# imagemagick/ImageMagick

Measured on NVIDIA H100. Metric: Mpixels/s on 8K RGBA Gaussian-blur σ=4 + Lanczos 2×; % HBM roofline, higher is better.
Workload: dtype f64

## Files before the change

### imagemagick_b200/csrc/conv_mma.cu

```cuda
#include "mb200_internal.h"
#include "conv_common.cuh"

#include <cuda_runtime.h>

#include <cstdint>

namespace mb200 {
namespace {

template <int NKS>
struct MmaTaps { double k[4 * NKS]; };

struct MmaArgs {
  const void *src;
  void *dst;
  int width, height;
  int off;
  int ntaps;
  int strip;
  const float *aux;
  double gain, qthreshold;
  int l2pf;
};

__device__ __forceinline__ void dmma(double (&d)[2], double a, double b) {
  asm volatile("mma.sync.aligned.m8n8k4.row.col.f64.f64.f64.f64 {%0,%1}, {%2}, {%3}, {%0,%1};"
      : "+d"(d[0]), "+d"(d[1]) : "d"(a), "d"(b));
}

template <int IO> struct Raw;
template <> struct Raw<0> { float4 a; };
template <> struct Raw<2> { double2 a, b; };

template <int NKS, int AXIS, int IO, int EPI, int MINB>
__global__ void __launch_bounds__(128, MINB) conv_mma_kernel(const MmaArgs a, const MmaTaps<NKS> taps) {
  static_assert(NKS % 2 == 0, "the prologue stages whole 8-position blocks");
  static_assert(EPI == 0 || (AXIS == 1 && IO == 0), "the fused epilogue belongs to the final column pass");
// ... 236 lines not shown
    output(prev, epi_prev, prev_valid);
    if (b > 0) outp += ostep;

    if (window_bad != 0) {
#pragma unroll
      for (int g = 0; g < 2; ++g) {
        double s0 = 0.0, s1 = 0.0, s2 = 0.0, s3 = 0.0;
        int u = 8 * sb + n8;
        if (u >= RR) u -= RR;
        for (int t = 0; t < a.ntaps; ++t) {
          const double *p = ring + static_cast<unsigned>(u) * kUStride + lane_px_off + g * kGroup;
          const double2 rg = *reinterpret_cast<const double2 *>(p);
          const double2 ba = *reinterpret_cast<const double2 *>(p + kBA);
          const double k = taps.k[t];
          s0 = fma(k, rg.x, s0); s1 = fma(k, rg.y, s1); s2 = fma(k, ba.x, s2); s3 = fma(k, ba.y, s3);
          if (++u == RR) u = 0;
        }
        acc[2 * g][0] = s0; acc[2 * g][1] = s1; acc[2 * g + 1][0] = s2; acc[2 * g + 1][1] = s3;
      }
    }
#pragma unroll
    for (int t = 0; t < 4; ++t) { prev[t][0] = acc[t][0]; prev[t][1] = acc[t][1]; }
    if (EPI) { epi_prev[0] = epi_cur[0]; epi_prev[1] = epi_cur[1]; }
    prev_valid = mvalid;
    st_slot = st_slot + 1 == NB ? 0 : st_slot + 1;
    if (++sb == NB) sb = 0;
  }
  output(prev, epi_prev, prev_valid);
}

template <int NKS>
struct WideTaps { double k[16 * NKS]; };

template <int NKS, int AXIS, int EPI>
__global__ void __launch_bounds__(128, 3) conv_mma_wide_kernel(const MmaArgs a, const WideTaps<NKS> taps) {
  static_assert(EPI == 0 || AXIS == 1, "the fused epilogue belongs to the final column pass");
  constexpr int NB = NKS + 1;
  constexpr int RR = 16 * NB;
  constexpr int PW = 36;
  constexpr int PL = 2 * RR + 8;
  constexpr int kWarpDoubles = AXIS == 1 ? RR * PW : 16 * PL;
  extern __shared__ __align__(16) double ring_all[];
  const int warp = threadIdx.x >> 5, lane = threadIdx.x & 31;
  double *ring = ring_all + warp * kWarpDoubles;
  const unsigned ring_s = static_cast<unsigned>(__cvta_generic_to_shared(ring));
  const int t4 = lane & 3, g8 = lane >> 2;

  int first, nout, limit, par0;
  if (AXIS == 1) {
    par0 = (blockIdx.x * 4 + warp) * 8;
    if (par0 >= a.width) return;
    first = blockIdx.y * a.strip;
    nout = min(a.strip, a.height - first);
    limit = a.height - 1;
  } else {
    par0 = (blockIdx.y * 4 + warp) * 8;
    if (par0 >= a.height) return;
    first = blockIdx.x * a.strip;
    nout = min(a.strip, a.width - first);
    limit = a.width - 1;
  }
  const int nblocks = (nout + 15) >> 4;
  const bool mma_l2pf = a.l2pf != 0;
  const size_t pitch = static_cast<size_t>(a.width) * 16;

  const int lq = lane & 7, lh = lane >> 3;
  const char *lbase[4];
  int uoff[4];
  unsigned st_off[4];
#pragma unroll
  for (int i = 0; i < 4; ++i) {
    if (AXIS == 1) {
      lbase[i] = static_cast<const char *>(a.src) + static_cast<size_t>(min(par0 + lq, a.width - 1)) * 16;
      uoff[i] = lh + 4 * i;
      st_off[i] = static_cast<unsigned>(uoff[i] * PW + 2 * lq);
    } else {
      const int line = lh + 4 * (i >> 1);
      lbase[i] = static_cast<const char *>(a.src) + static_cast<size_t>(min(par0 + line, a.height - 1)) * pitch;
      uoff[i] = lq + 8 * (i & 1);
      st_off[i] = static_cast<unsigned>(line * PL + 2 * uoff[i]);
    }
  }
  constexpr unsigned kBlockStride = AXIS == 1 ? 16 * PW : 32;
  constexpr unsigned kBA = AXIS == 1 ? 16 : 8 * PL;
  const size_t lstep = AXIS == 1 ? pitch : 16;
  const int base = first - a.off;

  float4 raw[4];
  auto fetch = [&](int j) {
#pragma unroll
    for (int i = 0; i < 4; ++i) {
      const unsigned pos = static_cast<unsigned>(min(max(base + 16 * j + uoff[i], 0), limit));
      raw[i] = __ldg(reinterpret_cast<const float4 *>(lbase[i] + static_cast<size_t>(pos) * lstep));
    }
  };
  constexpr int kL2Ahead = 4;
  auto prefetch_l2 = [&](int j) {
#pragma unroll
    for (int i = 0; i < 4; ++i) {
      const unsigned pos = static_cast<unsigned>(min(max(base + 16 * j + uoff[i], 0), limit));
      asm volatile("prefetch.global.L2 [%0];" ::"l"(lbase[i] + static_cast<size_t>(pos) * lstep));
    }
  };
  unsigned badmask = 0;
  auto stage = [&](int slot) {
    bool bad = false;
#pragma unroll
    for (int i = 0; i < 4; ++i) {
      const float4 f = raw[i];
      const unsigned m = max(max(__float_as_uint(f.x) & 0x7fffffffu, __float_as_uint(f.y) & 0x7fffffffu),
                             max(__float_as_uint(f.z) & 0x7fffffffu, __float_as_uint(f.w) & 0x7fffffffu));
      bad = bad || m >= 0x7f800000u;
      const double da = static_cast<double>(f.w);
      double *q = ring + st_off[i] + static_cast<unsigned>(slot) * kBlockStride;
      *reinterpret_cast<double2 *>(q) = make_double2(static_cast<double>(f.x) * da, static_cast<double>(f.y) * da);
      *reinterpret_cast<double2 *>(q + kBA) = make_double2(static_cast<double>(f.z) * da, da);
    }
    const bool any = __any_sync(0xffffffffu, bad);
    badmask = any ? (badmask | (1u << slot)) : (badmask & ~(1u << slot));
  };

  constexpr int NA = 4 * NKS + 2;
  double atap[NA];
#pragma unroll
  for (int c = 0; c < NA; ++c) {
    const int t = 4 * (c - 2) + t4 - g8;
    const double v = taps.k[min(max(t, 0), 16 * NKS - 1)];
    atap[c] = (t >= 0 && t < a.ntaps) ? v : 0.0;
  }

  const unsigned frag_off = AXIS == 1 ? static_cast<unsigned>(t4 * PW + g8)
                                      : static_cast<unsigned>(2 * t4 + (g8 >> 1) * PL + (g8 & 1));
  constexpr unsigned kUStride = AXIS == 1 ? PW : 2;
  constexpr unsigned kT2 = AXIS == 1 ? 8 : 4 * PL;
  constexpr unsigned kTile[4] = {0, kBA, kT2, kT2 + kBA};
  const unsigned lane_px_off = AXIS == 1 ? static_cast<unsigned>(2 * t4) : static_cast<unsigned>(t4 * PL);

  char *outp;
  if (AXIS == 1) {
    outp = static_cast<char *>(a.dst) + static_cast<size_t>(first + g8) * pitch + static_cast<size_t>(par0 + t4) * 16;
  } else {
    outp = static_cast<char *>(a.dst) + static_cast<size_t>(par0 + t4) * pitch + static_cast<size_t>(first + g8) * 16;
  }
  const size_t ostep = AXIS == 1 ? 16 * pitch : 16 * 16;
  const size_t gstep = AXIS == 1 ? 4 * 16 : 4 * pitch;
  const size_t hstep = AXIS == 1 ? 8 * pitch : 8 * 16;
  bool gvalid[2];
#pragma unroll
  for (int g = 0; g < 2; ++g) gvalid[g] = (par0 + 4 * g + t4) < (AXIS == 1 ? a.width : a.height);
  auto output = [&](const double (&acc)[4][4], const float4 (&epi)[2][2], int mrem) {
#pragma unroll
    for (int g = 0; g < 2; ++g)
#pragma unroll
      for (int h = 0; h < 2; ++h) {
        const double sr = acc[2 * g][2 * h], sg = acc[2 * g][2 * h + 1], sbv = acc[2 * g + 1][2 * h],
                     sa = acc[2 * g + 1][2 * h + 1];
        const double r = fast_reciprocal(clamp_denominator(sa));
        float4 out = make_float4(static_cast<float>(sr * r), static_cast<float>(sg * r), static_cast<float>(sbv * r),
                                 static_cast<float>(sa));
        if (EPI) {
          out.x = unsharp_point(epi[g][h].x, out.x, a.gain, a.qthreshold);
          out.y = unsharp_point(epi[g][h].y, out.y, a.gain, a.qthreshold);
          out.z = unsharp_point(epi[g][h].z, out.z, a.gain, a.qthreshold);
          out.w = unsharp_point(epi[g][h].w, out.w, a.gain, a.qthreshold);
        }
        if (g8 + 8 * h < mrem && gvalid[g]) *reinterpret_cast<float4 *>(outp + g * gstep + h * hstep) = out;
      }
  };

  {
    float4 pre[NKS][4];
#pragma unroll
    for (int j = 0; j < NKS; ++j) {
      fetch(j);
#pragma unroll
      for (int i = 0; i < 4; ++i) pre[j][i] = raw[i];
    }
#pragma unroll
    for (int j = 0; j < NKS; ++j) {
#pragma unroll
      for (int i = 0; i < 4; ++i) raw[i] = pre[j][i];
      stage(j);
    }
  }
  float4 ahead[4];
  fetch(NKS + 1);
#pragma unroll
  for (int i = 0; i < 4; ++i) ahead[i] = raw[i];
  fetch(NKS);

  int st_slot = NKS, sb = 0;
  double prev[4][4];
#pragma unroll
  for (int t = 0; t < 4; ++t)
#pragma unroll
    for (int i = 0; i < 4; ++i) prev[t][i] = (i & 1) ? 1.0 : 0.0;
  float4 epi_prev[2][2], epi_cur[2][2];
#pragma unroll
  for (int g = 0; g < 2; ++g)
#pragma unroll
    for (int h = 0; h < 2; ++h) epi_prev[g][h] = epi_cur[g][h] = make_float4(0.f, 0.f, 0.f, 0.f);
  int prev_rem = 0;

#pragma unroll 1
  for (int b = 0; b < nblocks; ++b) {
    __syncwarp();
    const int mrem = nout - 16 * b;
    const unsigned window_bad = badmask & ~(1u << st_slot);
    output(prev, epi_prev, prev_rem);
    if (b > 0) outp += ostep;
    if (EPI) {
      const char *epip = reinterpret_cast<const char *>(a.aux) + (outp - static_cast<char *>(a.dst));
#pragma unroll
      for (int g = 0; g < 2; ++g)
#pragma unroll
        for (int h = 0; h < 2; ++h)
          if (g8 + 8 * h < mrem && gvalid[g])
            epi_cur[g][h] = __ldg(reinterpret_cast<const float4 *>(epip + g * gstep + h * hstep));
    }
    stage(st_slot);
#pragma unroll
    for (int i = 0; i < 4; ++i) raw[i] = ahead[i];
    {
      float4 keep[4];
#pragma unroll
      for (int i = 0; i < 4; ++i) keep[i] = raw[i];
      fetch(b + NKS + 2);
      if (mma_l2pf) prefetch_l2(b + NKS + 2 + kL2Ahead);
#pragma unroll
      for (int i = 0; i < 4; ++i) { ahead[i] = raw[i]; raw[i] = keep[i]; }
    }
    double acc[4][4];
#pragma unroll
    for (int t = 0; t < 4; ++t)
#pragma unroll
      for (int i = 0; i < 4; ++i) acc[t][i] = 0.0;
    {
      unsigned ua[NKS];
#pragma unroll
      for (int s = 0; s < NKS; ++s) {
        const int blk = sb + s >= NB ? sb + s - NB : sb + s;
        ua[s] = ring_s + (frag_off + static_cast<unsigned>(blk) * kBlockStride) * 8u;
      }
      auto lds4 = [&](double (&bv)[4], int q) {
        const unsigned addr = ua[q >> 2] + kTile[q & 3] * 8;
#pragma unroll
        for (int i = 0; i < 4; ++i)
          asm volatile("ld.shared.f64 %0, [%1];" : "=d"(bv[i]) : "r"(addr + 4 * i * kUStride * 8));
      };
      double bq[2][4];
      lds4(bq[0], 0);
#pragma unroll
      for (int q = 0; q < 4 * NKS; ++q) {
        if (q + 1 < 4 * NKS) lds4(bq[(q + 1) & 1], q + 1);
        const double *av = atap + 4 * (q >> 2);
        double (&d)[4] = acc[q & 3];
        const double (&bv)[4] = bq[q & 1];
        asm volatile("mma.sync.aligned.m16n8k16.row.col.f64.f64.f64.f64 {%0,%1,%2,%3}, {%4,%5,%6,%7,%8,%9,%10,%11}, "
                     "{%12,%13,%14,%15}, {%0,%1,%2,%3};"
                     : "+d"(d[0]), "+d"(d[1]), "+d"(d[2]), "+d"(d[3])
                     : "d"(av[2]), "d"(av[0]), "d"(av[3]), "d"(av[1]), "d"(av[4]), "d"(av[2]), "d"(av[5]), "d"(av[3]),
                       "d"(bv[0]), "d"(bv[1]), "d"(bv[2]), "d"(bv[3]));
      }
    }
    if (window_bad != 0) {
#pragma unroll
      for (int g = 0; g < 2; ++g)
#pragma unroll
        for (int h = 0; h < 2; ++h) {
          double s0 = 0.0, s1 = 0.0, s2 = 0.0, s3 = 0.0;
          int u = 16 * sb + g8 + 8 * h;
          if (u >= RR) u -= RR;
          for (int t = 0; t < a.ntaps; ++t) {
            const double *p = ring + static_cast<unsigned>(u) * kUStride + lane_px_off + g * kT2;
            const double2 rg = *reinterpret_cast<const double2 *>(p);
            const double2 ba = *reinterpret_cast<const double2 *>(p + kBA);
            const double k = taps.k[t];
            s0 = fma(k, rg.x, s0); s1 = fma(k, rg.y, s1); s2 = fma(k, ba.x, s2); s3 = fma(k, ba.y, s3);
            if (++u == RR) u = 0;
          }
          acc[2 * g][2 * h] = s0; acc[2 * g][2 * h + 1] = s1; acc[2 * g + 1][2 * h] = s2; acc[2 * g + 1][2 * h + 1] = s3;
        }
    }
#pragma unroll
    for (int t = 0; t < 4; ++t)
#pragma unroll
      for (int i = 0; i < 4; ++i) prev[t][i] = acc[t][i];
    if (EPI) {
#pragma unroll
      for (int g = 0; g < 2; ++g)
#pragma unroll
        for (int h = 0; h < 2; ++h) epi_prev[g][h] = epi_cur[g][h];
    }
    prev_rem = mrem;
    st_slot = st_slot + 1 == NB ? 0 : st_slot + 1;
    if (++sb == NB) sb = 0;
  }
  output(prev, epi_prev, prev_rem);
}

template <int NKS, int AXIS, int EPI>
int launch_wide(const MmaArgs &a, const double *taps_host, cudaStream_t stream) {
  constexpr int RR = 16 * (NKS + 1);
  constexpr int kWarpDoubles = AXIS == 1 ? RR * 36 : 16 * (2 * RR + 8);
  constexpr size_t smem = 4 * kWarpDoubles * sizeof(double);
  WideTaps<NKS> taps;
  for (int i = 0; i < 16 * NKS; ++i) taps.k[i] = i < a.ntaps ? taps_host[i] : 0.0;
  dim3 grid;
  if (AXIS == 1) grid = dim3((a.width + 31) / 32, (a.height + a.strip - 1) / a.strip);
  else grid = dim3((a.width + a.strip - 1) / a.strip, (a.height + 31) / 32);
  if (grid.y > 65535) return MB200_EUNSUPPORTED;
  auto kernel = conv_mma_wide_kernel<NKS, AXIS, EPI>;
  if (smem > 48 * 1024) cudaFuncSetAttribute(kernel, cudaFuncAttributeMaxDynamicSharedMemorySize, static_cast<int>(smem));
  kernel<<<grid, 128, smem, stream>>>(a, taps);
  count_launch();
  count_family(kConvMma);
  count_family(kConvMmaWide);
  const cudaError_t e = cudaGetLastError();
  if (e != cudaSuccess) return cuda_fail(e, "conv_mma_wide launch");
  return MB200_OK;
}

template <int NKS>
int launch_wide_nks(const MmaArgs &a, const double *taps_host, int axis, bool epi, cudaStream_t stream) {
  if (axis == 0) return launch_wide<NKS, 0, 0>(a, taps_host, stream);
  if (epi) return launch_wide<NKS, 1, 1>(a, taps_host, stream);
  return launch_wide<NKS, 1, 0>(a, taps_host, stream);
}

template <int NKS, int AXIS, int IO, int EPI>
int launch_one(const MmaArgs &a, const MmaTaps<NKS> &taps, int minb, cudaStream_t stream) {
  constexpr int NB = (4 * NKS - 8) / 8 + 2, RR = 8 * NB;
  constexpr int kWarpDoubles = AXIS == 1 ? RR * 36 : 16 * (2 * RR + 8);
  constexpr size_t smem = 4 * kWarpDoubles * sizeof(double);
  dim3 grid;
  if (AXIS == 1) grid = dim3((a.width + 31) / 32, (a.height + a.strip - 1) / a.strip);
  else grid = dim3((a.width + a.strip - 1) / a.strip, (a.height + 31) / 32);
  if (grid.y > 65535) return MB200_EUNSUPPORTED;
  auto go = [&](auto kernel) {
    if (smem > 48 * 1024) cudaFuncSetAttribute(kernel, cudaFuncAttributeMaxDynamicSharedMemorySize, static_cast<int>(smem));
    kernel<<<grid, 128, smem, stream>>>(a, taps);
  };
  if (minb >= 4) go(conv_mma_kernel<NKS, AXIS, IO, EPI, 4>);
  else go(conv_mma_kernel<NKS, AXIS, IO, EPI, 3>);
  count_launch();
  count_family(kConvMma);
  const cudaError_t e = cudaGetLastError();
// ... 53 lines not shown
```

### imagemagick_b200/csrc/resize_stream.cu

```cuda
#include "mb200_internal.h"

#include <cuda.h>
#include <cudaTypedefs.h>
#include <cuda_runtime.h>

#include <algorithm>
#include <cstdlib>

namespace mb200 {
namespace {

constexpr double kQuantumScale = 1.0 / 65535.0;
constexpr double kEpsilon = 1.0e-12;
constexpr int kMaxSegments = MB200_RESIZE_MAX_SEGMENTS;

struct StreamArgs {
  const float *src;
  float *dst;
  int width, height;
  int out_w, out_h;
  int in_n;
  int strip;
  int nseg;
  int seg_o[kMaxSegments];
  int seg_n[kMaxSegments];
  int seg_src[kMaxSegments];
  int seg_strip0[kMaxSegments];
  const double *wsets;
  int nstrips;
  int nborder, out_n;
  const int *border;
  const int *start, *count;
  const double *weights;
};

__device__ __forceinline__ double fast_reciprocal(double g) {
// ... 203 lines not shown
  __syncwarp();
  unsigned rd = ring_s + lane * kRowPitch + px_in * 16;
  float4 vnext;
  asm volatile("ld.shared.v4.f32 {%0,%1,%2,%3}, [%4];" : "=f"(vnext.x), "=f"(vnext.y), "=f"(vnext.z), "=f"(vnext.w) : "r"(rd));
#pragma unroll 1
  for (int t = 0; t < niter; ++t) {
#pragma unroll
    for (int b = 0; b < BODY; ++b) {
      const int m = b % P;
      const float4 v = vnext;
      rd += 16;
      if (++px_in == kChunkPx) {
        px_in = 0;
        __syncwarp();
        issue(chunk + NSLOT);
        ++chunk;
        cp_async_wait<NSLOT - 1>();
        __syncwarp();
        rd = ring_s + static_cast<unsigned>(chunk % NSLOT) * kSlotBytes + lane * kRowPitch;
      }
      asm volatile("ld.shared.v4.f32 {%0,%1,%2,%3}, [%4];" : "=f"(vnext.x), "=f"(vnext.y), "=f"(vnext.z), "=f"(vnext.w) : "r"(rd));
      feed<S, N>(acc, W, v, m);
      const int qd = done_slot<S, N>(m);
      if (qd >= 0) {
        ++c;
        if (c >= 0 && c < st.nout && active) *reinterpret_cast<float4 *>(outp) = finish_rgba(acc[qd]);
        outp += 4;
      }
    }
  }
  cp_async_wait<0>();
}

__device__ __forceinline__ void mbar_init(unsigned bar, unsigned count) {
  asm volatile("mbarrier.init.shared::cta.b64 [%0], %1;" ::"r"(bar), "r"(count));
}
__device__ __forceinline__ void mbar_expect_tx(unsigned bar, unsigned bytes) {
  asm volatile("mbarrier.arrive.expect_tx.shared::cta.b64 _, [%0], %1;" ::"r"(bar), "r"(bytes) : "memory");
}
__device__ __forceinline__ void mbar_wait(unsigned bar, unsigned parity) {
  asm volatile(
      "{\n"
      ".reg .pred p;\n"
      "MB200_WAIT:\n"
      "mbarrier.try_wait.parity.shared::cta.b64 p, [%0], %1;\n"
      "@p bra MB200_DONE;\n"
      "bra MB200_WAIT;\n"
      "MB200_DONE:\n"
      "}\n" ::"r"(bar), "r"(parity) : "memory");
}
__device__ __forceinline__ void tma_load_2d(unsigned dst, const CUtensorMap *map, int c0, int c1, unsigned bar) {
  asm volatile("cp.async.bulk.tensor.2d.shared::cluster.global.mbarrier::complete_tx::bytes [%0], [%1, {%2, %3}], [%4];"
               ::"r"(dst), "l"(map), "r"(c0), "r"(c1), "r"(bar) : "memory");
}

template <int S, int N, int NSLOT, int MINB, int BOXES = 2>
__global__ void __launch_bounds__(128, MINB) resize_h_tma_kernel(const StreamArgs a, const __grid_constant__ CUtensorMap tmap) {
  using T = Rot<S, N>;
  constexpr int kChunkPx = 8 * BOXES, kBoxBytes = 32 * 128, kSlotBytes = BOXES * kBoxBytes;
  constexpr int R = T::R, P = T::P, BODY = T::BODY;
  extern __shared__ __align__(1024) unsigned char ring_all[];
  __shared__ __align__(8) unsigned long long bars[4][NSLOT];
  const int warp = threadIdx.x >> 5, lane = threadIdx.x & 31;
  const unsigned ring_base = (static_cast<unsigned>(__cvta_generic_to_shared(ring_all)) + 1023u) & ~1023u;
  const unsigned ring_s = ring_base + static_cast<unsigned>(warp) * NSLOT * kSlotBytes;
  const unsigned bar_s = static_cast<unsigned>(__cvta_generic_to_shared(&bars[warp][0]));
  const int row0 = blockIdx.y * 128 + warp * 32;
  if (row0 >= a.height) return;
  if (static_cast<int>(blockIdx.x) >= a.nstrips) {
    if (row0 + lane < a.height) border_output<0>(a, __ldg(a.border + (blockIdx.x - a.nstrips)), row0 + lane);
    return;
  }
  const Strip st = locate(a, blockIdx.x, S);
  double W[N];
#pragma unroll
  for (int j = 0; j < N; ++j) W[j] = __ldg(a.wsets + st.set * N + j);
  const int niter = (S * (st.nout - 1) + N + BODY - 1) / BODY;
  const int p0 = st.src0;
  const int c0 = p0 / kChunkPx;
  const int nchunks = (p0 + S * (st.nout - 1) + N + kChunkPx - 1) / kChunkPx - c0;
  if (lane == 0) {
#pragma unroll
    for (int k = 0; k < NSLOT; ++k) mbar_init(bar_s + 8 * k, 1);
    asm volatile("fence.mbarrier_init.release.cluster;" ::: "memory");
  }
  __syncwarp();
  auto issue = [&](int chunk_rel) {
    if (lane == 0 && chunk_rel < nchunks) {
// ... 21 lines not shown
  const unsigned row_off = lane * 128, swz = lane & 7;
  auto addr = [&](unsigned slot, int p) {
    return slot + static_cast<unsigned>(p >> 3) * kBoxBytes + row_off + ((static_cast<unsigned>(p & 7) ^ swz) << 4);
  };
  mbar_wait(bar_s, 0);
  unsigned slot_s = ring_s;
  float4 vnext;
  asm volatile("ld.shared.v4.f32 {%0,%1,%2,%3}, [%4];" : "=f"(vnext.x), "=f"(vnext.y), "=f"(vnext.z), "=f"(vnext.w) : "r"(addr(slot_s, px_in)));
#pragma unroll 1
  for (int t = 0; t < niter; ++t) {
#pragma unroll
    for (int b = 0; b < BODY; ++b) {
      const int m = b % P;
      const float4 v = vnext;
      if (++px_in == kChunkPx) {
        px_in = 0;
        __syncwarp();
        issue(chunk + NSLOT);
        ++chunk;
        const int k = chunk % NSLOT;
        if (chunk < nchunks) mbar_wait(bar_s + 8 * k, static_cast<unsigned>(chunk / NSLOT) & 1u);
        slot_s = ring_s + static_cast<unsigned>(k) * kSlotBytes;
      }
      asm volatile("ld.shared.v4.f32 {%0,%1,%2,%3}, [%4];" : "=f"(vnext.x), "=f"(vnext.y), "=f"(vnext.z), "=f"(vnext.w) : "r"(addr(slot_s, px_in)));
      feed<S, N>(acc, W, v, m);
      const int qd = done_slot<S, N>(m);
      if (qd >= 0) {
        ++c;
        if (c >= 0 && c < st.nout && active) *reinterpret_cast<float4 *>(outp) = finish_rgba(acc[qd]);
        outp += 4;
      }
    }
  }
}

bool make_row_tensor_map(const float *src, int width, int height, CUtensorMap *map) {
  static PFN_cuTensorMapEncodeTiled encode = [] {
    void *fn = nullptr;
    cudaDriverEntryPointQueryResult q;
    if (cudaGetDriverEntryPoint("cuTensorMapEncodeTiled", &fn, cudaEnableDefault, &q) != cudaSuccess ||
        q != cudaDriverEntryPointSuccess)
      fn = nullptr;
    return reinterpret_cast<PFN_cuTensorMapEncodeTiled>(fn);
  }();
  if (encode == nullptr) return false;
  const cuuint64_t dims[2] = {static_cast<cuuint64_t>(width) * 4, static_cast<cuuint64_t>(height)};
  const cuuint64_t strides[1] = {static_cast<cuuint64_t>(width) * 16};
  const cuuint32_t box[2] = {32, 32}, estr[2] = {1, 1};
  return encode(map, CU_TENSOR_MAP_DATA_TYPE_FLOAT32, 2, const_cast<float *>(src), dims, strides, box, estr,
                CU_TENSOR_MAP_INTERLEAVE_NONE, CU_TENSOR_MAP_SWIZZLE_128B, CU_TENSOR_MAP_L2_PROMOTION_L2_256B,
                CU_TENSOR_MAP_FLOAT_OOB_FILL_NONE) == CUDA_SUCCESS;
}

struct Tile { int o0, nout, src0, set; };
struct FusedArgs {
  const float *src;
  float *dst;
  int width, height, out_w, out_h;
  const Tile *xt, *yt;
  const double *wx, *wy;
};

template <int S, int N>
constexpr bool fused_fits(int nw) {
  return S * (4 * nw - 1) + N <= 128 &&
         S * 3 * nw + ((S * (nw - 1) + N + Rot<S, N>::BODY - 1) / Rot<S, N>::BODY) * Rot<S, N>::BODY + 1 <= 128;
}
template <int S, int N>
constexpr int fused_nw() {
  int nw = 13;
  while (nw > 1 && !fused_fits<S, N>(nw)) --nw;
  return nw;
}

template <int S, int N> struct FusedGeom {
  static constexpr int P = Rot<S, N>::P;
  static constexpr int TH = 31;
  static constexpr int NW = fused_nw<S, N>();
  static_assert(fused_fits<S, N>(NW), "no phase-B split fits the 128-column tile");
  static constexpr int TW = 4 * NW;
  static constexpr int PF = Rot<S, N>::PF == 12 ? 6 : Rot<S, N>::PF;
  static constexpr int kPitch = 128 * 16 + 16;
  static constexpr int kSmem = 32 * kPitch;
};
// ... 185 lines not shown
    resize_border2d_kernel<<<dim3(static_cast<unsigned>((work + 127) / 128), 2), 128, 0, s>>>(b, y.d_is_border);
    count_launch();
  }
  const cudaError_t e = cudaGetLastError();
  if (e != cudaSuccess) return cuda_fail(e, "fused resize launch");
  return MB200_OK;
}

namespace {

template <int S, int N>
int launch_sn(StreamArgs a, int axis, cudaStream_t s) {
  const TuningKnobs knobs = tuning_knobs();
  const int lanes_blocks = axis == 1 ? (a.width + 127) / 128 : (a.height + 127) / 128;
  int total = 0;
  for (int k = 0; k < a.nseg; ++k) total += a.seg_n[k];
  const int want = (8 * sm_count() * 3 + lanes_blocks - 1) / lanes_blocks;
  int strip = (total + want - 1) / want;
  if (strip < 24) strip = 24;
  if (knobs.resize_strip > 0) strip = knobs.resize_strip;
  a.strip = strip;
  int nstrips = 0;
  for (int k = 0; k < a.nseg; ++k) {
    a.seg_strip0[k] = nstrips;
    nstrips += (a.seg_n[k] + strip - 1) / strip;
  }
  a.nstrips = nstrips;
  nstrips += a.nborder;
  if (nstrips <= 0 || nstrips > 65535 || lanes_blocks > 65535) return MB200_EUNSUPPORTED;
  const int tma = knobs.resize_tma, chunk = knobs.resize_chunk, slots = knobs.resize_slots;
  LaunchFamily family = kResizeHStream;
  CUtensorMap tmap;
  if (axis == 0 && tma != 0 && (reinterpret_cast<uintptr_t>(a.src) & 15) == 0 &&
      make_row_tensor_map(a.src, a.width, a.height, &tmap)) {
    family = kResizeHTma;
    if (tma == 2) {
      constexpr int smem = 4 * 2 * 8192 + 1024;
      cudaFuncSetAttribute(resize_h_tma_kernel<S, N, 2, 3>, cudaFuncAttributeMaxDynamicSharedMemorySize, smem);
      resize_h_tma_kernel<S, N, 2, 3><<<dim3(nstrips, lanes_blocks), 128, smem, s>>>(a, tmap);
    } else {
      constexpr int smem = 4 * 3 * 8192 + 1024;
      cudaFuncSetAttribute(resize_h_tma_kernel<S, N, 3, 2>, cudaFuncAttributeMaxDynamicSharedMemorySize, smem);
      resize_h_tma_kernel<S, N, 3, 2><<<dim3(nstrips, lanes_blocks), 128, smem, s>>>(a, tmap);
    }
  } else if (axis == 1) {
    family = kResizeVStream;
    resize_v_stream_kernel<S, N><<<dim3(lanes_blocks, nstrips), 128, 0, s>>>(a);
  } else if (chunk == 16 && slots == 2) {
    constexpr int smem = 4 * 2 * HRing<16>::kSlotBytes;
    cudaFuncSetAttribute(resize_h_stream_kernel<S, N, 2, 3, 16>, cudaFuncAttributeMaxDynamicSharedMemorySize, smem);
    resize_h_stream_kernel<S, N, 2, 3, 16><<<dim3(nstrips, lanes_blocks), 128, smem, s>>>(a);
  } else if (chunk == 16) {
    constexpr int smem = 4 * 3 * HRing<16>::kSlotBytes;
    cudaFuncSetAttribute(resize_h_stream_kernel<S, N, 3, 2, 16>, cudaFuncAttributeMaxDynamicSharedMemorySize, smem);
    resize_h_stream_kernel<S, N, 3, 2, 16><<<dim3(nstrips, lanes_blocks), 128, smem, s>>>(a);
  } else if (slots == 3) {
    constexpr int smem = 4 * 3 * HRing<8>::kSlotBytes;
    cudaFuncSetAttribute(resize_h_stream_kernel<S, N, 3, 4, 8>, cudaFuncAttributeMaxDynamicSharedMemorySize, smem);
    resize_h_stream_kernel<S, N, 3, 4, 8><<<dim3(nstrips, lanes_blocks), 128, smem, s>>>(a);
  } else {
    constexpr int smem = 4 * 4 * HRing<8>::kSlotBytes;
    cudaFuncSetAttribute(resize_h_stream_kernel<S, N, 4, 3, 8>, cudaFuncAttributeMaxDynamicSharedMemorySize, smem);
    resize_h_stream_kernel<S, N, 4, 3, 8><<<dim3(nstrips, lanes_blocks), 128, smem, s>>>(a);
  }
  count_family(family);
  return MB200_OK;
}
// ... 36 lines not shown
```

Baseline: 26310.

## Feed wide MMA convolution through per-warp TMA ring and persistent tile scheduling

Each warp now pulls its 16-position input boxes through a 4-stage TMA/mbarrier ring in shared memory instead of per-lane __ldg loads with register lookahead and L2 prefetch. The grid becomes persistent, sized to two CTAs per SM, and each warp walks a contiguous range of (band, strip) tiles so consecutive strips in a band can share staging. The intent is to hide global load latency with asynchronous bulk copies and to cut launch tail effects. In exchange shared memory per CTA grows, occupancy drops from 3 to 2 CTAs per SM, and the kernel now depends on tensor map encoding succeeding. TMA helpers move into a shared header.

```diff
diff --git a/imagemagick_b200/csrc/conv_mma.cu b/imagemagick_b200/csrc/conv_mma.cu
--- a/imagemagick_b200/csrc/conv_mma.cu
+++ b/imagemagick_b200/csrc/conv_mma.cu
@@ -1,8 +1,10 @@
 #include "mb200_internal.h"
 #include "conv_common.cuh"
+#include "tma.cuh"
 
 #include <cuda_runtime.h>
 
+#include <algorithm>
 #include <cstdint>
 
 namespace mb200 {
@@ -305,75 +307,116 @@
 template <int NKS>
 struct WideTaps { double k[16 * NKS]; };
 
+constexpr int kWideStages = 4;
+constexpr unsigned kWideBoxBytes = 2048;
+
 template <int NKS, int AXIS, int EPI>
-__global__ void __launch_bounds__(128, 3) conv_mma_wide_kernel(const MmaArgs a, const WideTaps<NKS> taps) {
+__global__ void __launch_bounds__(128, 2) conv_mma_wide_kernel(const MmaArgs a, const WideTaps<NKS> taps,
+                                                                const __grid_constant__ CUtensorMap tmap) {
   static_assert(EPI == 0 || AXIS == 1, "the fused epilogue belongs to the final column pass");
   constexpr int NB = NKS + 1;
   constexpr int RR = 16 * NB;
   constexpr int PW = 36;
   constexpr int PL = 2 * RR + 8;
   constexpr int kWarpDoubles = AXIS == 1 ? RR * PW : 16 * PL;
-  extern __shared__ __align__(16) double ring_all[];
+  constexpr int W = 4, S = kWideStages;
+  extern __shared__ __align__(128) unsigned char smem_all[];
+  __shared__ __align__(8) unsigned long long bars[W][S];
   const int warp = threadIdx.x >> 5, lane = threadIdx.x & 31;
-  double *ring = ring_all + warp * kWarpDoubles;
+  unsigned char *smem = smem_all + ((128u - (static_cast<unsigned>(__cvta_generic_to_shared(smem_all)) & 127u)) & 127u);
+  const unsigned raw_s = static_cast<unsigned>(__cvta_generic_to_shared(smem)) + warp * S * kWideBoxBytes;
+  double *ring = reinterpret_cast<double *>(smem + W * S * kWideBoxBytes) + warp * kWarpDoubles;
   const unsigned ring_s = static_cast<unsigned>(__cvta_generic_to_shared(ring));
+  const unsigned bar_s = static_cast<unsigned>(__cvta_generic_to_shared(&bars[warp][0]));
   const int t4 = lane & 3, g8 = lane >> 2;
 
-  int first, nout, limit, par0;
-  if (AXIS == 1) {
-    par0 = (blockIdx.x * 4 + warp) * 8;
-    if (par0 >= a.width) return;
-    first = blockIdx.y * a.strip;
-    nout = min(a.strip, a.height - first);
-    limit = a.height - 1;
-  } else {
-    par0 = (blockIdx.y * 4 + warp) * 8;
-    if (par0 >= a.height) return;
-    first = blockIdx.x * a.strip;
-    nout = min(a.strip, a.width - first);
-    limit = a.width - 1;
-  }
-  const int nblocks = (nout + 15) >> 4;
-  const bool mma_l2pf = a.l2pf != 0;
-  const size_t pitch = static_cast<size_t>(a.width) * 16;
+  const int len = AXIS == 1 ? a.height : a.width;
+  const int limit = len - 1;
+  const int nstrips = (len + a.strip - 1) / a.strip;
+  const long long ntiles = static_cast<long long>(((AXIS == 1 ? a.width : a.height) + 7) >> 3) * nstrips;
+  const long long nwarps = static_cast<long long>(gridDim.x) * W, gw = static_cast<long long>(blockIdx.x) * W + warp;
+  const long long per = ntiles / nwarps, extra = ntiles % nwarps;
+  const long long t_begin = gw * per + min(gw, extra), t_end = t_begin + per + (gw < extra ? 1 : 0);
+  if (t_begin >= t_end) return;
+  struct Seg { long long end; int band, first, nout; };
+  auto segment = [&](long long t) {
+    Seg sg;
+    sg.band = static_cast<int>(t / nstrips);
+    const long long band_end = static_cast<long long>(sg.band + 1) * nstrips;
+    sg.end = min(t_end, band_end);
+    sg.first = static_cast<int>(t - static_cast<long long>(sg.band) * nstrips) * a.strip;
+    sg.nout = min(static_cast<int>(sg.end - static_cast<long long>(sg.band) * nstrips) * a.strip, len) - sg.first;
+    return sg;
+  };
+  auto box_start = [&](int p0) { return min(max(p0, 0), max(limit - 15, 0)); };
+
+  if (lane == 0) {
+#pragma unroll
+    for (int k = 0; k < S; ++k) mbar_init(bar_s + 8 * k, 1);
+    asm volatile("fence.mbarrier_init.release.cluster;" ::: "memory");
+  }
+  __syncwarp();
+
+  Seg pseg = segment(t_begin);
+  int pj = 0;
+  unsigned np = 0, nc = 0;
+  auto issue_next = [&]() {
+    if (pseg.band < 0) return;
+    const int s0 = box_start(pseg.first - a.off + 16 * pj);
+    if (lane == 0) {
+      const unsigned k = np % S, bar = bar_s + 8 * k;
+      asm volatile("fence.proxy.async.shared::cta;" ::: "memory");
+      mbar_expect_tx(bar, kWideBoxBytes);
+      if (AXIS == 1) tma_load_2d(raw_s + k * kWideBoxBytes, &tmap, pseg.band * 32, s0, bar);
+      else tma_load_2d(raw_s + k * kWideBoxBytes, &tmap, s0 * 4, pseg.band * 8, bar);
+    }
+    ++np;
+    if (++pj == ((pseg.nout + 15) >> 4) + NKS - 1) {
+      pj = 0;
+      if (pseg.end < t_end) pseg = segment(pseg.end);
+      else pseg.band = -1;
+    }
+  };
+#pragma unroll
+  for (int k = 0; k < S; ++k) issue_next();
 
   const int lq = lane & 7, lh = lane >> 3;
-  const char *lbase[4];
   int uoff[4];
+  unsigned raw_off[4];
   unsigned st_off[4];
 #pragma unroll
   for (int i = 0; i < 4; ++i) {
     if (AXIS == 1) {
-      lbase[i] = static_cast<const char *>(a.src) + static_cast<size_t>(min(par0 + lq, a.width - 1)) * 16;
       uoff[i] = lh + 4 * i;
+      raw_off[i] = static_cast<unsigned>(lq * 16);
       st_off[i] = static_cast<unsigned>(uoff[i] * PW + 2 * lq);
     } else {
       const int line = lh + 4 * (i >> 1);
-      lbase[i] = static_cast<const char *>(a.src) + static_cast<size_t>(min(par0 + line, a.height - 1)) * pitch;
       uoff[i] = lq + 8 * (i & 1);
+      raw_off[i] = static_cast<unsigned>(line * 256);
       st_off[i] = static_cast<unsigned>(line * PL + 2 * uoff[i]);
     }
   }
+  constexpr unsigned kPosBytes = AXIS == 1 ? 128 : 16;
   constexpr unsigned kBlockStride = AXIS == 1 ? 16 * PW : 32;
   constexpr unsigned kBA = AXIS == 1 ? 16 : 8 * PL;
-  const size_t lstep = AXIS == 1 ? pitch : 16;
-  const int base = first - a.off;
 
   float4 raw[4];
-  auto fetch = [&](int j) {
+  int base = 0;
+  auto take = [&](int j) {
+    const unsigned k = nc % S;
+    mbar_wait(bar_s + 8 * k, (nc / S) & 1u);
+    const int p0 = base + 16 * j, s0 = box_start(p0);
 #pragma unroll
     for (int i = 0; i < 4; ++i) {
-      const unsigned pos = static_cast<unsigned>(min(max(base + 16 * j + uoff[i], 0), limit));
-      raw[i] = __ldg(reinterpret_cast<const float4 *>(lbase[i] + static_cast<size_t>(pos) * lstep));
-    }
-  };
-  constexpr int kL2Ahead = 4;
-  auto prefetch_l2 = [&](int j) {
-#pragma unroll
-    for (int i = 0; i < 4; ++i) {
-      const unsigned pos = static_cast<unsigned>(min(max(base + 16 * j + uoff[i], 0), limit));
-      asm volatile("prefetch.global.L2 [%0];" ::"l"(lbase[i] + static_cast<size_t>(pos) * lstep));
-    }
+      const unsigned pos = static_cast<unsigned>(min(max(p0 + uoff[i], 0), limit) - s0);
+      const unsigned addr = raw_s + k * kWideBoxBytes + raw_off[i] + pos * kPosBytes;
+      asm volatile("ld.shared.v4.f32 {%0,%1,%2,%3}, [%4];"
+                   : "=f"(raw[i].x), "=f"(raw[i].y), "=f"(raw[i].z), "=f"(raw[i].w) : "r"(addr) : "memory");
+    }
+    ++nc;
+    __syncwarp();
+    issue_next();
   };
   unsigned badmask = 0;
   auto stage = [&](int slot) {
@@ -409,183 +452,177 @@
   constexpr unsigned kTile[4] = {0, kBA, kT2, kT2 + kBA};
   const unsigned lane_px_off = AXIS == 1 ? static_cast<unsigned>(2 * t4) : static_cast<unsigned>(t4 * PL);
 
-  char *outp;
-  if (AXIS == 1) {
-    outp = static_cast<char *>(a.dst) + static_cast<size_t>(first + g8) * pitch + static_cast<size_t>(par0 + t4) * 16;
-  } else {
-    outp = static_cast<char *>(a.dst) + static_cast<size_t>(par0 + t4) * pitch + static_cast<size_t>(first + g8) * 16;
-  }
+  const size_t pitch = static_cast<size_t>(a.width) * 16;
   const size_t ostep = AXIS == 1 ? 16 * pitch : 16 * 16;
   const size_t gstep = AXIS == 1 ? 4 * 16 : 4 * pitch;
   const size_t hstep = AXIS == 1 ? 8 * pitch : 8 * 16;
-  bool gvalid[2];
-#pragma unroll
-  for (int g = 0; g < 2; ++g) gvalid[g] = (par0 + 4 * g + t4) < (AXIS == 1 ? a.width : a.height);
-  auto output = [&](const double (&acc)[4][4], const float4 (&epi)[2][2], int mrem) {
+
+#pragma unroll 1
+  for (long long tile = t_begin; tile < t_end;) {
+    const Seg sg = segment(tile);
+    tile = sg.end;
+    const int par0 = sg.band * 8, first = sg.first, nout = sg.nout;
+    const int nblocks = (nout + 15) >> 4;
+    base = first - a.off;
+
+    char *outp;
+    if (AXIS == 1) {
+      outp = static_cast<char *>(a.dst) + static_cast<size_t>(first + g8) * pitch + static_cast<size_t>(par0 + t4) * 16;
+    } else {
+      outp = static_cast<char *>(a.dst) + static_cast<size_t>(par0 + t4) * pitch + static_cast<size_t>(first + g8) * 16;
+    }
+    bool gvalid[2];
+#pragma unroll
+    for (int g = 0; g < 2; ++g) gvalid[g] = (par0 + 4 * g + t4) < (AXIS == 1 ? a.width : a.height);
+    auto output = [&](const double (&acc)[4][4], const float4 (&epi)[2][2], int mrem) {
+#pragma unroll
+      for (int g = 0; g < 2; ++g)
+#pragma unroll
+        for (int h = 0; h < 2; ++h) {
+          const double sr = acc[2 * g][2 * h], sg = acc[2 * g][2 * h + 1], sbv = acc[2 * g + 1][2 * h],
+                       sa = acc[2 * g + 1][2 * h + 1];
+          const double r = fast_reciprocal(clamp_denominator(sa));
+          float4 out = make_float4(static_cast<float>(sr * r), static_cast<float>(sg * r), static_cast<float>(sbv * r),
+                                   static_cast<float>(sa));
+          if (EPI) {
+            out.x = unsharp_point(epi[g][h].x, out.x, a.gain, a.qthreshold);
+            out.y = unsharp_point(epi[g][h].y, out.y, a.gain, a.qthreshold);
+            out.z = unsharp_point(epi[g][h].z, out.z, a.gain, a.qthreshold);
+            out.w = unsharp_point(epi[g][h].w, out.w, a.gain, a.qthreshold);
+          }
+          if (g8 + 8 * h < mrem && gvalid[g]) *reinterpret_cast<float4 *>(outp + g * gstep + h * hstep) = out;
+        }
+    };
+
+    badmask = 0;
+#pragma unroll
+    for (int j = 0; j < NKS; ++j) {
+      take(j);
+      stage(j);
+    }
+    if (nblocks > 1) take(NKS);
+
+    int st_slot = NKS, sb = 0;
+    double prev[4][4];
+#pragma unroll
+    for (int t = 0; t < 4; ++t)
+#pragma unroll
+      for (int i = 0; i < 4; ++i) prev[t][i] = (i & 1) ? 1.0 : 0.0;
+    float4 epi_prev[2][2], epi_cur[2][2];
 #pragma unroll
     for (int g = 0; g < 2; ++g)
 #pragma unroll
-      for (int h = 0; h < 2; ++h) {
-        const double sr = acc[2 * g][2 * h], sg = acc[2 * g][2 * h + 1], sbv = acc[2 * g + 1][2 * h],
-                     sa = acc[2 * g + 1][2 * h + 1];
-        const double r = fast_reciprocal(clamp_denominator(sa));
-        float4 out = make_float4(static_cast<float>(sr * r), static_cast<float>(sg * r), static_cast<float>(sbv * r),
-                                 static_cast<float>(sa));
-        if (EPI) {
-          out.x = unsharp_point(epi[g][h].x, out.x, a.gain, a.qthreshold);
-          out.y = unsharp_point(epi[g][h].y, out.y, a.gain, a.qthreshold);
-          out.z = unsharp_point(epi[g][h].z, out.z, a.gain, a.qthreshold);
-          out.w = unsharp_point(epi[g][h].w, out.w, a.gain, a.qthreshold);
+      for (int h = 0; h < 2; ++h) epi_prev[g][h] = epi_cur[g][h] = make_float4(0.f, 0.f, 0.f, 0.f);
+    int prev_rem = 0;
+
+#pragma unroll 1
+    for (int b = 0; b < nblocks; ++b) {
+      __syncwarp();
+      const int mrem = nout - 16 * b;
+      const unsigned window_bad = badmask & ~(1u << st_slot);
+      output(prev, epi_prev, prev_rem);
+      if (b > 0) outp += ostep;
+      if (EPI) {
+        const char *epip = reinterpret_cast<const char *>(a.aux) + (outp - static_cast<char *>(a.dst));
+#pragma unroll
+        for (int g = 0; g < 2; ++g)
+#pragma unroll
+          for (int h = 0; h < 2; ++h)
+            if (g8 + 8 * h < mrem && gvalid[g])
+              epi_cur[g][h] = __ldg(reinterpret_cast<const float4 *>(epip + g * gstep + h * hstep));
+      }
+      if (b + 1 < nblocks) stage(st_slot);
+      double acc[4][4];
+#pragma unroll
+      for (int t = 0; t < 4; ++t)
+#pragma unroll
+        for (int i = 0; i < 4; ++i) acc[t][i] = 0.0;
+      {
+        unsigned ua[NKS];
+#pragma unroll
+        for (int s = 0; s < NKS; ++s) {
+          const int blk = sb + s >= NB ? sb + s - NB : sb + s;
+          ua[s] = ring_s + (frag_off + static_cast<unsigned>(blk) * kBlockStride) * 8u;
         }
-        if (g8 + 8 * h < mrem && gvalid[g]) *reinterpret_cast<float4 *>(outp + g * gstep + h * hstep) = out;
-      }
-  };
-
-  {
-    float4 pre[NKS][4];
-#pragma unroll
-    for (int j = 0; j < NKS; ++j) {
-      fetch(j);
-#pragma unroll
-      for (int i = 0; i < 4; ++i) pre[j][i] = raw[i];
-    }
-#pragma unroll
-    for (int j = 0; j < NKS; ++j) {
-#pragma unroll
-      for (int i = 0; i < 4; ++i) raw[i] = pre[j][i];
-      stage(j);
-    }
-  }
-  float4 ahead[4];
-  fetch(NKS + 1);
-#pragma unroll
-  for (int i = 0; i < 4; ++i) ahead[i] = raw[i];
-  fetch(NKS);
-
-  int st_slot = NKS, sb = 0;
-  double prev[4][4];
-#pragma unroll
-  for (int t = 0; t < 4; ++t)
-#pragma unroll
-    for (int i = 0; i < 4; ++i) prev[t][i] = (i & 1) ? 1.0 : 0.0;
-  float4 epi_prev[2][2], epi_cur[2][2];
-#pragma unroll
-  for (int g = 0; g < 2; ++g)
-#pragma unroll
-    for (int h = 0; h < 2; ++h) epi_prev[g][h] = epi_cur[g][h] = make_float4(0.f, 0.f, 0.f, 0.f);
-  int prev_rem = 0;
-
-#pragma unroll 1
-  for (int b = 0; b < nblocks; ++b) {
-    __syncwarp();
-    const int mrem = nout - 16 * b;
-    const unsigned window_bad = badmask & ~(1u << st_slot);
+        auto lds4 = [&](double (&bv)[4], int q) {
+          const unsigned addr = ua[q >> 2] + kTile[q & 3] * 8;
+#pragma unroll
+          for (int i = 0; i < 4; ++i)
+            asm volatile("ld.shared.f64 %0, [%1];" : "=d"(bv[i]) : "r"(addr + 4 * i * kUStride * 8));
+        };
+        double bq[2][4];
+        lds4(bq[0], 0);
+#pragma unroll
+        for (int q = 0; q < 4 * NKS; ++q) {
+          if (q + 1 < 4 * NKS) lds4(bq[(q + 1) & 1], q + 1);
+          const double *av = atap + 4 * (q >> 2);
+          double (&d)[4] = acc[q & 3];
+          const double (&bv)[4] = bq[q & 1];
+          asm volatile("mma.sync.aligned.m16n8k16.row.col.f64.f64.f64.f64 {%0,%1,%2,%3}, {%4,%5,%6,%7,%8,%9,%10,%11}, "
+                       "{%12,%13,%14,%15}, {%0,%1,%2,%3};"
+                       : "+d"(d[0]), "+d"(d[1]), "+d"(d[2]), "+d"(d[3])
+                       : "d"(av[2]), "d"(av[0]), "d"(av[3]), "d"(av[1]), "d"(av[4]), "d"(av[2]), "d"(av[5]), "d"(av[3]),
+                         "d"(bv[0]), "d"(bv[1]), "d"(bv[2]), "d"(bv[3]));
+        }
+      }
+      if (b + 2 < nblocks) take(b + NKS + 1);
+      if (window_bad != 0) {
+#pragma unroll
+        for (int g = 0; g < 2; ++g)
+#pragma unroll
+          for (int h = 0; h < 2; ++h) {
+            double s0 = 0.0, s1 = 0.0, s2 = 0.0, s3 = 0.0;
+            int u = 16 * sb + g8 + 8 * h;
+            if (u >= RR) u -= RR;
+            for (int t = 0; t < a.ntaps; ++t) {
+              const double *p = ring + static_cast<unsigned>(u) * kUStride + lane_px_off + g * kT2;
+              const double2 rg = *reinterpret_cast<const double2 *>(p);
+              const double2 ba = *reinterpret_cast<const double2 *>(p + kBA);
+              const double k = taps.k[t];
+              s0 = fma(k, rg.x, s0); s1 = fma(k, rg.y, s1); s2 = fma(k, ba.x, s2); s3 = fma(k, ba.y, s3);
+              if (++u == RR) u = 0;
+            }
+            acc[2 * g][2 * h] = s0; acc[2 * g][2 * h + 1] = s1; acc[2 * g + 1][2 * h] = s2; acc[2 * g + 1][2 * h + 1] = s3;
+          }
+      }
+#pragma unroll
+      for (int t = 0; t < 4; ++t)
+#pragma unroll
+        for (int i = 0; i < 4; ++i) prev[t][i] = acc[t][i];
+      if (EPI) {
+#pragma unroll
+        for (int g = 0; g < 2; ++g)
+#pragma unroll
+          for (int h = 0; h < 2; ++h) epi_prev[g][h] = epi_cur[g][h];
+      }
+      prev_rem = mrem;
+      st_slot = st_slot + 1 == NB ? 0 : st_slot + 1;
+      if (++sb == NB) sb = 0;
+    }
     output(prev, epi_prev, prev_rem);
-    if (b > 0) outp += ostep;
-    if (EPI) {
-      const char *epip = reinterpret_cast<const char *>(a.aux) + (outp - static_cast<char *>(a.dst));
-#pragma unroll
-      for (int g = 0; g < 2; ++g)
-#pragma unroll
-        for (int h = 0; h < 2; ++h)
-          if (g8 + 8 * h < mrem && gvalid[g])
-            epi_cur[g][h] = __ldg(reinterpret_cast<const float4 *>(epip + g * gstep + h * hstep));
-    }
-    stage(st_slot);
-#pragma unroll
-    for (int i = 0; i < 4; ++i) raw[i] = ahead[i];
-    {
-      float4 keep[4];
-#pragma unroll
-      for (int i = 0; i < 4; ++i) keep[i] = raw[i];
-      fetch(b + NKS + 2);
-      if (mma_l2pf) prefetch_l2(b + NKS + 2 + kL2Ahead);
-#pragma unroll
-      for (int i = 0; i < 4; ++i) { ahead[i] = raw[i]; raw[i] = keep[i]; }
-    }
-    double acc[4][4];
-#pragma unroll
-    for (int t = 0; t < 4; ++t)
-#pragma unroll
-      for (int i = 0; i < 4; ++i) acc[t][i] = 0.0;
-    {
-      unsigned ua[NKS];
-#pragma unroll
-      for (int s = 0; s < NKS; ++s) {
-        const int blk = sb + s >= NB ? sb + s - NB : sb + s;
-        ua[s] = ring_s + (frag_off + static_cast<unsigned>(blk) * kBlockStride) * 8u;
-      }
-      auto lds4 = [&](double (&bv)[4], int q) {
-        const unsigned addr = ua[q >> 2] + kTile[q & 3] * 8;
-#pragma unroll
-        for (int i = 0; i < 4; ++i)
-          asm volatile("ld.shared.f64 %0, [%1];" : "=d"(bv[i]) : "r"(addr + 4 * i * kUStride * 8));
-      };
-      double bq[2][4];
-      lds4(bq[0], 0);
-#pragma unroll
-      for (int q = 0; q < 4 * NKS; ++q) {
-        if (q + 1 < 4 * NKS) lds4(bq[(q + 1) & 1], q + 1);
-        const double *av = atap + 4 * (q >> 2);
-        double (&d)[4] = acc[q & 3];
-        const double (&bv)[4] = bq[q & 1];
-        asm volatile("mma.sync.aligned.m16n8k16.row.col.f64.f64.f64.f64 {%0,%1,%2,%3}, {%4,%5,%6,%7,%8,%9,%10,%11}, "
-                     "{%12,%13,%14,%15}, {%0,%1,%2,%3};"
-                     : "+d"(d[0]), "+d"(d[1]), "+d"(d[2]), "+d"(d[3])
-                     : "d"(av[2]), "d"(av[0]), "d"(av[3]), "d"(av[1]), "d"(av[4]), "d"(av[2]), "d"(av[5]), "d"(av[3]),
-                       "d"(bv[0]), "d"(bv[1]), "d"(bv[2]), "d"(bv[3]));
-      }
-    }
-    if (window_bad != 0) {
-#pragma unroll
-      for (int g = 0; g < 2; ++g)
-#pragma unroll
-        for (int h = 0; h < 2; ++h) {
-          double s0 = 0.0, s1 = 0.0, s2 = 0.0, s3 = 0.0;
-          int u = 16 * sb + g8 + 8 * h;
-          if (u >= RR) u -= RR;
-          for (int t = 0; t < a.ntaps; ++t) {
-            const double *p = ring + static_cast<unsigned>(u) * kUStride + lane_px_off + g * kT2;
-            const double2 rg = *reinterpret_cast<const double2 *>(p);
-            const double2 ba = *reinterpret_cast<const double2 *>(p + kBA);
-            const double k = taps.k[t];
-            s0 = fma(k, rg.x, s0); s1 = fma(k, rg.y, s1); s2 = fma(k, ba.x, s2); s3 = fma(k, ba.y, s3);
-            if (++u == RR) u = 0;
-          }
-          acc[2 * g][2 * h] = s0; acc[2 * g][2 * h + 1] = s1; acc[2 * g + 1][2 * h] = s2; acc[2 * g + 1][2 * h + 1] = s3;
-        }
-    }
-#pragma unroll
-    for (int t = 0; t < 4; ++t)
-#pragma unroll
-      for (int i = 0; i < 4; ++i) prev[t][i] = acc[t][i];
-    if (EPI) {
-#pragma unroll
-      for (int g = 0; g < 2; ++g)
-#pragma unroll
-        for (int h = 0; h < 2; ++h) epi_prev[g][h] = epi_cur[g][h];
-    }
-    prev_rem = mrem;
-    st_slot = st_slot + 1 == NB ? 0 : st_slot + 1;
-    if (++sb == NB) sb = 0;
-  }
-  output(prev, epi_prev, prev_rem);
+  }
 }
 
 template <int NKS, int AXIS, int EPI>
 int launch_wide(const MmaArgs &a, const double *taps_host, cudaStream_t stream) {
   constexpr int RR = 16 * (NKS + 1);
   constexpr int kWarpDoubles = AXIS == 1 ? RR * 36 : 16 * (2 * RR + 8);
-  constexpr size_t smem = 4 * kWarpDoubles * sizeof(double);
+  constexpr size_t smem = 4 * (kWarpDoubles * sizeof(double) + kWideStages * kWideBoxBytes) + 128;
   WideTaps<NKS> taps;
   for (int i = 0; i < 16 * NKS; ++i) taps.k[i] = i < a.ntaps ? taps_host[i] : 0.0;
-  dim3 grid;
-  if (AXIS == 1) grid = dim3((a.width + 31) / 32, (a.height + a.strip - 1) / a.strip);
-  else grid = dim3((a.width + a.strip - 1) / a.strip, (a.height + 31) / 32);
-  if (grid.y > 65535) return MB200_EUNSUPPORTED;
+  constexpr int kCtasPerSm = 2;
+  static_assert(kCtasPerSm * (smem + 1024) <= 228 * 1024, "two CTAs' rings must fit in an SM's shared memory");
+  CUtensorMap tmap;
+  if (!make_rgba_tensor_map(static_cast<const float *>(a.src), a.width, a.height, AXIS == 1 ? 32 : 64, AXIS == 1 ? 16 : 8,
+                            CU_TENSOR_MAP_SWIZZLE_NONE,
+                            AXIS == 1 ? CU_TENSOR_MAP_L2_PROMOTION_L2_128B : CU_TENSOR_MAP_L2_PROMOTION_L2_256B, &tmap))
+    return MB200_EUNSUPPORTED;
   auto kernel = conv_mma_wide_kernel<NKS, AXIS, EPI>;
-  if (smem > 48 * 1024) cudaFuncSetAttribute(kernel, cudaFuncAttributeMaxDynamicSharedMemorySize, static_cast<int>(smem));
-  kernel<<<grid, 128, smem, stream>>>(a, taps);
+  cudaFuncSetAttribute(kernel, cudaFuncAttributeMaxDynamicSharedMemorySize, static_cast<int>(smem));
+  const long long lines = AXIS == 1 ? a.width : a.height, len = AXIS == 1 ? a.height : a.width;
+  const long long tiles = (lines + 7) / 8 * ((len + a.strip - 1) / a.strip);
+  const int grid = static_cast<int>(std::min<long long>(static_cast<long long>(kCtasPerSm) * sm_count(), (tiles + 3) / 4));
+  kernel<<<grid, 128, smem, stream>>>(a, taps, tmap);
   count_launch();
   count_family(kConvMma);
   count_family(kConvMmaWide);
diff --git a/imagemagick_b200/csrc/resize_stream.cu b/imagemagick_b200/csrc/resize_stream.cu
--- a/imagemagick_b200/csrc/resize_stream.cu
+++ b/imagemagick_b200/csrc/resize_stream.cu
@@ -1,7 +1,7 @@
 #include "mb200_internal.h"
 
-#include <cuda.h>
-#include <cudaTypedefs.h>
+#include "tma.cuh"
+
 #include <cuda_runtime.h>
 
 #include <algorithm>
@@ -271,28 +271,6 @@
   cp_async_wait<0>();
 }
 
-__device__ __forceinline__ void mbar_init(unsigned bar, unsigned count) {
-  asm volatile("mbarrier.init.shared::cta.b64 [%0], %1;" ::"r"(bar), "r"(count));
-}
-__device__ __forceinline__ void mbar_expect_tx(unsigned bar, unsigned bytes) {
-  asm volatile("mbarrier.arrive.expect_tx.shared::cta.b64 _, [%0], %1;" ::"r"(bar), "r"(bytes) : "memory");
-}
-__device__ __forceinline__ void mbar_wait(unsigned bar, unsigned parity) {
-  asm volatile(
-      "{\n"
-      ".reg .pred p;\n"
-      "MB200_WAIT:\n"
-      "mbarrier.try_wait.parity.shared::cta.b64 p, [%0], %1;\n"
-      "@p bra MB200_DONE;\n"
-      "bra MB200_WAIT;\n"
-      "MB200_DONE:\n"
-      "}\n" ::"r"(bar), "r"(parity) : "memory");
-}
-__device__ __forceinline__ void tma_load_2d(unsigned dst, const CUtensorMap *map, int c0, int c1, unsigned bar) {
-  asm volatile("cp.async.bulk.tensor.2d.shared::cluster.global.mbarrier::complete_tx::bytes [%0], [%1, {%2, %3}], [%4];"
-               ::"r"(dst), "l"(map), "r"(c0), "r"(c1), "r"(bar) : "memory");
-}
-
 template <int S, int N, int NSLOT, int MINB, int BOXES = 2>
 __global__ void __launch_bounds__(128, MINB) resize_h_tma_kernel(const StreamArgs a, const __grid_constant__ CUtensorMap tmap) {
   using T = Rot<S, N>;
@@ -380,24 +358,6 @@
       }
     }
   }
-}
-
-bool make_row_tensor_map(const float *src, int width, int height, CUtensorMap *map) {
-  static PFN_cuTensorMapEncodeTiled encode = [] {
-    void *fn = nullptr;
-    cudaDriverEntryPointQueryResult q;
-    if (cudaGetDriverEntryPoint("cuTensorMapEncodeTiled", &fn, cudaEnableDefault, &q) != cudaSuccess ||
-        q != cudaDriverEntryPointSuccess)
-      fn = nullptr;
-    return reinterpret_cast<PFN_cuTensorMapEncodeTiled>(fn);
-  }();
-  if (encode == nullptr) return false;
-  const cuuint64_t dims[2] = {static_cast<cuuint64_t>(width) * 4, static_cast<cuuint64_t>(height)};
-  const cuuint64_t strides[1] = {static_cast<cuuint64_t>(width) * 16};
-  const cuuint32_t box[2] = {32, 32}, estr[2] = {1, 1};
-  return encode(map, CU_TENSOR_MAP_DATA_TYPE_FLOAT32, 2, const_cast<float *>(src), dims, strides, box, estr,
-                CU_TENSOR_MAP_INTERLEAVE_NONE, CU_TENSOR_MAP_SWIZZLE_128B, CU_TENSOR_MAP_L2_PROMOTION_L2_256B,
-                CU_TENSOR_MAP_FLOAT_OOB_FILL_NONE) == CUDA_SUCCESS;
 }
 
 struct Tile { int o0, nout, src0, set; };
@@ -649,7 +609,8 @@
   LaunchFamily family = kResizeHStream;
   CUtensorMap tmap;
   if (axis == 0 && tma != 0 && (reinterpret_cast<uintptr_t>(a.src) & 15) == 0 &&
-      make_row_tensor_map(a.src, a.width, a.height, &tmap)) {
+      make_rgba_tensor_map(a.src, a.width, a.height, 32, 32, CU_TENSOR_MAP_SWIZZLE_128B,
+                           CU_TENSOR_MAP_L2_PROMOTION_L2_256B, &tmap)) {
     family = kResizeHTma;
     if (tma == 2) {
       constexpr int smem = 4 * 2 * 8192 + 1024;
diff --git a/imagemagick_b200/csrc/tma.cuh b/imagemagick_b200/csrc/tma.cuh
--- /dev/null
+++ b/imagemagick_b200/csrc/tma.cuh
@@ -0,0 +1,50 @@
+#pragma once
+
+#include <cuda.h>
+#include <cudaTypedefs.h>
+#include <cuda_runtime.h>
+
+namespace mb200 {
+
+__device__ __forceinline__ void mbar_init(unsigned bar, unsigned count) {
+  asm volatile("mbarrier.init.shared::cta.b64 [%0], %1;" ::"r"(bar), "r"(count));
+}
+__device__ __forceinline__ void mbar_expect_tx(unsigned bar, unsigned bytes) {
+  asm volatile("mbarrier.arrive.expect_tx.shared::cta.b64 _, [%0], %1;" ::"r"(bar), "r"(bytes) : "memory");
+}
+__device__ __forceinline__ void mbar_wait(unsigned bar, unsigned parity) {
+  asm volatile(
+      "{\n"
+      ".reg .pred p;\n"
+      "MB200_WAIT:\n"
+      "mbarrier.try_wait.parity.shared::cta.b64 p, [%0], %1;\n"
+      "@p bra MB200_DONE;\n"
+      "bra MB200_WAIT;\n"
+      "MB200_DONE:\n"
+      "}\n" ::"r"(bar), "r"(parity) : "memory");
+}
+__device__ __forceinline__ void tma_load_2d(unsigned dst, const CUtensorMap *map, int c0, int c1, unsigned bar) {
+  asm volatile("cp.async.bulk.tensor.2d.shared::cluster.global.mbarrier::complete_tx::bytes [%0], [%1, {%2, %3}], [%4];"
+               ::"r"(dst), "l"(map), "r"(c0), "r"(c1), "r"(bar) : "memory");
+}
+
+inline bool make_rgba_tensor_map(const float *src, int width, int height, unsigned box_floats, unsigned box_rows,
+                                 CUtensorMapSwizzle swizzle, CUtensorMapL2promotion promotion, CUtensorMap *map) {
+  static PFN_cuTensorMapEncodeTiled encode = [] {
+    void *fn = nullptr;
+    cudaDriverEntryPointQueryResult q;
+    if (cudaGetDriverEntryPoint("cuTensorMapEncodeTiled", &fn, cudaEnableDefault, &q) != cudaSuccess ||
+        q != cudaDriverEntryPointSuccess)
+      fn = nullptr;
+    return reinterpret_cast<PFN_cuTensorMapEncodeTiled>(fn);
+  }();
+  if (encode == nullptr) return false;
+  const cuuint64_t dims[2] = {static_cast<cuuint64_t>(width) * 4, static_cast<cuuint64_t>(height)};
+  const cuuint64_t strides[1] = {static_cast<cuuint64_t>(width) * 16};
+  const cuuint32_t box[2] = {box_floats, box_rows}, estr[2] = {1, 1};
+  return encode(map, CU_TENSOR_MAP_DATA_TYPE_FLOAT32, 2, const_cast<float *>(src), dims, strides, box, estr,
+                CU_TENSOR_MAP_INTERLEAVE_NONE, swizzle, promotion,
+                CU_TENSOR_MAP_FLOAT_OOB_FILL_NONE) == CUDA_SUCCESS;
+}
+
+}
```

Result: faster. 27810 (median of 6 runs) (+5.7%).
